# adi-gov-tw/Taiwan-Tongues-ASR-CE

Measured on AMD Instinct MI355X. Metric: audio-sec/s (RTF) whisper-large-v3 greedy, 30 s clips, batch 32; 1/2/4/8 GPU, higher is better.
Workload: dtype bf16

## Files before the change

taiwan_tongues_asr_ce_amd/csrc/common.hpp:

```cpp
#pragma once
#include <hip/hip_runtime.h>
#include <stdint.h>

typedef uint16_t bf16_t;

using f32x4 = __attribute__((ext_vector_type(4))) float;
using f32x16 = __attribute__((ext_vector_type(16))) float;
using s16x8 = __attribute__((ext_vector_type(8))) short;
using s16x4 = __attribute__((ext_vector_type(4))) short;

__device__ __forceinline__ float bf2f(bf16_t v) { return __uint_as_float(((uint32_t)v) << 16); }
__device__ __forceinline__ bf16_t f2bf(float f) { return __builtin_bit_cast(bf16_t, (__bf16)f); }
__device__ __forceinline__ uint32_t f2bf_pk(float lo, float hi) {
  typedef __bf16 bf16x2_hw __attribute__((ext_vector_type(2)));
  typedef float f32x2_hw __attribute__((ext_vector_type(2)));
  return __builtin_bit_cast(uint32_t, __builtin_convertvector((f32x2_hw){lo, hi}, bf16x2_hw));
}
struct f16_t { uint16_t bits; };
using h16x8 = __attribute__((ext_vector_type(8))) _Float16;
typedef _Float16 h16x2_hw __attribute__((ext_vector_type(2)));

template <typename T> struct N16;
template <> struct N16<bf16_t> {
  static __device__ __forceinline__ float up(uint16_t b) { return __uint_as_float(((uint32_t)b) << 16); }
// ... 198 lines not shown
                const float* filters , const float* dft_cos, const float* dft_sin ,
                const float* window , float* logmel , unsigned* clip_max ,
                hipStream_t s, const int64_t* geom_dev = nullptr);
unsigned mel_max_to_ordered(float v);
float mel_max_from_ordered(unsigned u);
template <typename T>
void launch_mel_finish(float* logmel, const unsigned* clip_max, T* mel_t , int B, int n_mels,
                       int n_frames, hipStream_t s, const int64_t* geom_dev = nullptr);
template <typename T>
void launch_mel_transpose(const float* mel, T* mel_t, int B, int n_mels, int n_frames, hipStream_t s);

template <typename T> void launch_enc_attn_simple(const T* qkv, T* out, int B, int T_, int H, hipStream_t s);
template <typename T16> void launch_enc_attn_flash_bf16(const T16* qkv, T16* out, int B, int T_, int H, hipStream_t s);
template <typename T16>
void launch_cross_attn_flash_bf16(const T16* q, const T16* K, const T16* V, T16* out, int n_clips, int n_q, int H, int Tk, hipStream_t s);

struct RuleDyn { int32_t max_prompt, max_new, sot_index; uint32_t seed; };
struct DecState {
  int32_t* cur_tok;
  int32_t* step;
  int32_t* n_sampled;
  int32_t* last_tok;
  int32_t* pen_tok;
  int32_t* last_ts;
  int32_t* done;
  int32_t* n_done;
  float* sum_logprob;
  float* no_speech;
  int32_t* out_tokens;
  const int32_t* prompt;
  const int32_t* prompt_len;
  const uint8_t* mask;
  const RuleDyn* dyn;
  const int32_t* row_cap;
};
struct RuleParams {
  int V, ldv, max_prompt, max_new;
  int eot, no_timestamps, timestamp_begin, no_speech, sot_index, timestamps, max_initial, suppress_eot;
  float temperature;
  uint32_t seed;
};
template <typename T>
void launch_cross_attn_probs(const T* q, const T* K, const T* V, T* out, int rows, int H, int Tk, const int* sel ,
                             float* probs , hipStream_t s);
void launch_token_logprob(const float* logits, int ldv, int V, const int32_t* target, float* out, int rows, hipStream_t s);
void launch_token_prob(const float* logits, int ldv, int V, int tok, float* out , int rows, hipStream_t s);
template <typename T>
void launch_embed_prefill(const int32_t* prompt, int max_prompt, int rows_per_prompt, int n_seq, int npos, const T* emb, const T* pos,
                          float* x, int d, hipStream_t s);
template <typename T>
void launch_self_attn_prefill(const T* qkv , T* kv_pool, const int32_t* page_table, int pages_per_seq,
                              int64_t pool_layer_off, int identity_pages, T* out, int n_seq, int npos, int H, hipStream_t s);
template <typename T>
void launch_self_attn_decode(const T* qkv , T* kv_pool, const int32_t* page_table, int pages_per_seq,
                             int64_t pool_layer_off, int identity_pages, int row0, const int32_t* step, T* out , int B, int H,
                             hipStream_t s, SlabIn sq = SlabIn{} ,
                             const int32_t* done = nullptr );
template <typename T>
void launch_self_attn_decode_rows(const T* qkv, T* kv_pool, const int32_t* page_table, int pages_per_seq, int64_t pool_layer_off,
                                  int identity_pages, int row0, const int32_t* row_pos, T* out, int B, int H, hipStream_t s, SlabIn sq,
                                  const int32_t* done);
template <typename T>
void launch_copy_pages(T* pool, const int32_t* pairs_dev, int n_pairs, int n_layers, int H, int64_t layer_elems, hipStream_t s);
template <typename T>
void launch_cross_attn_decode(const T* q , const T* K, const T* V , T* out, int B, int H,
                              int Tk, int kv_div, hipStream_t s,
                              float* split_ws = nullptr ,
                              SlabIn sq = SlabIn{} ,
                              int ws_rows = 0 ,
                              QProj qp = QProj{} ,
                              const int32_t* done = nullptr );
template <typename T> void launch_xkv_quant(const T* src, uint8_t* dst, float* scale, int64_t n_blocks, int rows, hipStream_t s);
template <typename T>
bool launch_cross_attn_fp8(const T* q, const uint8_t* K8, const uint8_t* V8, const float* kscale, const float* vscale, T* out, int B, int H,
                           int Tk, hipStream_t s, struct SlabIn sq, const int32_t* done = nullptr);
extern thread_local bool g_kernel_sig_on;
extern thread_local char g_kernel_sig[192];
template <typename T> inline const char* sig_type() { return sizeof(T) == 4 ? "float" : "unsigned short"; }
template <> inline const char* sig_type<struct f16_t>() { return "f16_t"; }

extern thread_local char g_launch_fault[160];
void launch_fault(const char* fmt, ...);
extern thread_local int g_skinny_x_lds;
extern thread_local int g_skinny_nt;
extern thread_local int g_xattn_variant;
extern thread_local int g_flash_qw;
extern thread_local int g_xattn_mq_slices;
extern thread_local int g_xattn_deep_items;
struct BeamRowState { const int32_t *n_sampled, *last_tok, *pen_tok, *last_ts; const uint8_t* mask; };
void launch_beam_topk(const float* logits, BeamRowState st, RuleParams rp, int R, int k, float* out_lp ,
                      int32_t* out_id , float* out_no_speech , hipStream_t s);
void launch_select(const float* logits, DecState st, RuleParams rp, int B, float* out_rows , hipStream_t s,
                   int32_t* ticket, int total_rows);
void launch_advance(int32_t* step, hipStream_t s);
void launch_select_rows(const float* logits, DecState st, RuleParams rp, int B, hipStream_t s);
void launch_admit_rows(const int32_t* tab, int n, int B, int max_prompt, DecState st, int32_t* prompt, int32_t* prompt_len, int32_t* row_cap,
                       int32_t* row_pos, hipStream_t s);
void launch_prep_weight(const void* src, int src_type , float* dst, int64_t n, int64_t conv_in, float scale,
                        hipStream_t s);
template <typename T> void launch_cast(const float* in, T* out, int64_t n, hipStream_t s);
template <typename T> void launch_uncast(const T* in, float* out, int64_t n, hipStream_t s);
```

taiwan_tongues_asr_ce_amd/csrc/engine_ctx.hpp:

```cpp
#pragma once
#include <hip/hip_runtime.h>

#include <cmath>
#include <cstdarg>
#include <cstdio>
#include <cstdlib>
#include <cstring>
#include <algorithm>
#include <atomic>
#include <map>
#include <memory>
#include <mutex>
#include <string>
#include <unordered_map>
#include <vector>

#include "../../include/ttasr.h"
#include "common.hpp"

namespace ttasr_detail {


extern thread_local std::string g_create_error;

// ... 24 lines not shown
  int device = 0;
  hipStream_t stream = nullptr;
  hipStream_t cur = nullptr;
  std::string err;
  bool lowp = false;
  bool f16 = false;
  bool finalized = false;
  bool force_basic = false;
  bool use_graph = true;
  size_t esz = 4;
  int T = 0, F = 0, d = 0, H = 0, ffn = 0, V = 0, ldv = 0, M = 0, maxB = 0, n_samples = 0;
  int pages_per_seq = 0;
  std::vector<void*> allocs;
  struct Pool { char* base = nullptr; size_t cap = 0, used = 0; } small_pool, big_pool;
  size_t arena_hint = 0;
  std::unordered_map<std::string, Slot> slots;

  void *conv1_w = nullptr, *conv2_w = nullptr, *emb = nullptr, *dpos = nullptr, *emb_sh = nullptr;
  float *conv1_b = nullptr, *conv2_b = nullptr, *epos = nullptr, *elnf_g = nullptr, *elnf_b = nullptr, *dlnf_g = nullptr,
        *dlnf_b = nullptr;
  std::vector<EncLayerW> enc;
  std::vector<DecLayerW> dec;
  float* stage_f32 = nullptr;
  float* stage_raw = nullptr;
  size_t stage_elems = 0;

  float *filters = nullptr, *dcos = nullptr, *dsin = nullptr, *window = nullptr;

  float* pcm_dev = nullptr; int64_t* nsamp_dev = nullptr; unsigned* clip_max = nullptr; int64_t* mel_geom = nullptr;
  float* mel = nullptr; void* mel_t = nullptr; void* c1 = nullptr;
  float* x = nullptr; void *h = nullptr, *qkv = nullptr, *att = nullptr, *mid = nullptr, *enc_out = nullptr;
  void* xkv = nullptr; int64_t xkv_layer_elems = 0, xkv_which_elems = 0;
  bool xkv_fp8 = false, xkv8_valid = false; uint8_t* xkv8 = nullptr; float* xkv8_scale = nullptr;
  void* pool = nullptr; int64_t pool_layer_elems = 0; int32_t* page_table = nullptr;
  float* xsplit_ws = nullptr;
  float* dx = nullptr; void *dh = nullptr, *dqkv = nullptr, *dq = nullptr, *datt = nullptr, *dmid = nullptr; float* logits = nullptr;
  float* rows_out = nullptr;
  int kv_div = 1;
  int identity_pages = 1;
  int32_t* pairs_dev = nullptr;
  float* topk_lp = nullptr; int32_t* topk_id = nullptr; int32_t* row_state = nullptr;
#ifdef TTASR_EXPERIMENTS
  int skip_mask = 0;
#else
  static constexpr int skip_mask = 0;
#endif
  float* slab = nullptr;
  int ks_want[4] = {0, 0, 0, 0};
  int gemm_force = 0;
  bool gemm_persistent = true;
  bool vocab_persistent = true;
  bool no_flash = false;
  int prefill_ns_min = 2;
  bool enc_res_epilogue = false;
  DecState st{}; int32_t* prompt_dev = nullptr; int32_t* plen_dev = nullptr; uint8_t* mask_dev = nullptr;
  ttasr_ctx* weight_owner = nullptr;
  std::atomic<int> sharers{0};
  bool destroy_pending = false;
  int32_t* row_cap_dev = nullptr;
  int flash_qw = 2;
  int xattn_mq_slices = 0;
  int xattn_deep_items = 512;
  bool ragged_exit = true;
  RuleDyn* rule_dyn_dev = nullptr; RuleDyn rule_dyn_host{};
  int32_t* pinned_i32 = nullptr;
  char* pinned_beam = nullptr; size_t pinned_beam_bytes = 0;
  float beam_prof_ms[4]{0, 0, 0, 0};
  int max_new_alloc = 0, max_prompt_alloc = 0;

  ttasr_detail::Session* sess = nullptr;
  bool session_rows = false;
  bool refill_overlap = false;
  int32_t* row_pos = nullptr;
  void* xkv_stage = nullptr;
  int32_t* admit_dev = nullptr;

  int B_mel = 0, B_enc = 0, B_dec = 0;
  std::atomic_flag busy = ATOMIC_FLAG_INIT;
  int xattn_nt = 1, xattn_pipe = 1, weights_nt = 1;
  bool dec_narrow = true;
  bool weights_packed = false;
  bool enc_ln_defer = true;
  bool dec_x_lds = true;
  bool gemm_tail = true;
  bool xkv_grouped = true;
  bool multi_step = true;
  bool no_xsplit = false;
  bool no_prefill = false;
  bool prefill_tiled = false;
  hipEvent_t ev[8]{};
  std::string bench_sig;
  float phase_ms[4]{0, 0, 0, 0};
  bool enc_timing = false;
  std::vector<hipEvent_t> enc_ev;
  std::vector<int> enc_ev_class;
  float enc_class_ms[8]{0, 0, 0, 0, 0, 0, 0, 0};

  struct GraphKey { int B; int mode; int variant; hipGraphExec_t exec; };
  std::vector<GraphKey> graphs;
  static constexpr size_t kMaxGraphs = 32;
  RuleParams rp{};
};

namespace ttasr_detail {

int fail(ttasr_ctx* c, int code, const char* fmt, ...);

#define HIPCHK(c, call)                                                                                       \
  do {                                                                                                        \
    hipError_t e_ = (call);                                                                                   \
    if (e_ != hipSuccess) return fail((c), TTASR_E_HIP, "%s failed: %s (%s:%d)", #call, hipGetErrorString(e_), \
                                      __FILE__, __LINE__);                                                    \
  } while (0)


template <class F>
inline int guarded(ttasr_ctx* c, F&& f) {
  struct Busy {
    ttasr_ctx* c; bool own;
    explicit Busy(ttasr_ctx* c_) : c(c_), own(c_ == nullptr || !c_->busy.test_and_set(std::memory_order_acquire)) {}
    ~Busy() { if (c && own) c->busy.clear(std::memory_order_release); }
  } busy(c);
  if (!busy.own) return TTASR_E_INVALID;
  if (c) { g_xattn_variant = c->xattn_nt | (c->xattn_pipe << 1); g_skinny_nt = c->weights_nt; g_skinny_narrow = c->dec_narrow ? 1 : 0; g_skinny_x_lds = c->dec_x_lds ? 1 : 0; g_xattn_deep_items = c->xattn_deep_items; g_xattn_mq_slices = c->xattn_mq_slices; g_flash_qw = c->flash_qw; }
  g_launch_fault[0] = 0;
  try {
    const int rc = f();
    if (g_launch_fault[0] && rc == TTASR_OK) return fail(c, TTASR_E_INVALID, "launcher refused: %s", g_launch_fault);
    return rc;
  } catch (const std::bad_alloc&) {
    return fail(c, TTASR_E_NOMEM, "host allocation failed");
  } catch (const std::exception& e) {
    return fail(c, TTASR_E_INVALID, "C++ exception: %s", e.what());
  } catch (...) {
    return fail(c, TTASR_E_INVALID, "unknown C++ exception");
  }
}

template <typename P>
int dalloc(ttasr_ctx* c, P** p, size_t bytes, bool zero = true) {
  if (bytes == 0) bytes = 16;
  bytes = (bytes + 255) & ~(size_t)255;
  ttasr_ctx::Pool& pool = bytes < (1u << 20) ? c->small_pool : c->big_pool;
  const size_t big_chunk = c->arena_hint >= ((size_t)1 << 30) ? (size_t)1 << 30 : (size_t)64 << 20;
  const size_t chunk = &pool == &c->small_pool ? (size_t)64 << 20 : big_chunk;
  if (bytes > chunk / 2) {
    void* q = nullptr;
    hipError_t e = hipMalloc(&q, bytes);
    if (e != hipSuccess) return fail(c, TTASR_E_NOMEM, "hipMalloc(%zu) failed: %s", bytes, hipGetErrorString(e));
    c->allocs.push_back(q);
    if (zero) HIPCHK(c, hipMemsetAsync(q, 0, bytes, c->stream));
    *p = (P*)q;
    return 0;
  }
  if (pool.used + bytes > pool.cap) {
    void* q = nullptr;
    hipError_t e = hipMalloc(&q, chunk);
    if (e != hipSuccess) return fail(c, TTASR_E_NOMEM, "hipMalloc(%zu) failed: %s", chunk, hipGetErrorString(e));
    c->allocs.push_back(q);
    pool.base = (char*)q; pool.cap = chunk; pool.used = 0;
  }
  void* q = pool.base + pool.used;
  pool.used += bytes;
  if (zero) HIPCHK(c, hipMemsetAsync(q, 0, bytes, c->stream));
  *p = (P*)q;
  return 0;
}
#define TRY(expr) do { int rc_ = (expr); if (rc_ != 0) return rc_; } while (0)
#define TT_DISPATCH(c_, CALL)                                   \
  do {                                                          \
    if (!(c_)->lowp) { using T = float; CALL; }                 \
    else if ((c_)->f16) { using T = f16_t; CALL; }              \
    else { using T = bf16_t; CALL; }                            \
  } while (0)

template <typename T>
GemmArgs lin_args(const void* A, const void* W, int M, int N, int K) {
  GemmArgs g; g.A = A; g.W = W; g.M = M; g.N = N; g.K = K; g.lda = K; g.ldw = K; g.epi.ldc = N;
  return g;
}

enum EncClass { EC_CONV = 0, EC_LN = 1, EC_QKV = 2, EC_ATTN = 3, EC_OUT = 4, EC_FC1 = 5, EC_FC2 = 6, EC_XKV = 7 };
struct AlignOut {
  int clip;
  const int* sel;
  float* probs;
};

int build_weights(ttasr_ctx* c);
int build_workspaces(ttasr_ctx* c);
int ingest_tensor(ttasr_ctx* c, const char* name, const void* src, int src_type, const int64_t* dims, int32_t ndim);

void enc_mark(ttasr_ctx* c, int cls);
void sched_encoder(ttasr_ctx* c, int B);
void sched_cross_kv(ttasr_ctx* c, int B);
void sched_prefill(ttasr_ctx* c, int n_seq, int npos, int seq_per_clip, int max_prompt, const AlignOut* al = nullptr);
int sched_prefill_no_speech(ttasr_ctx* c, int n_seq, int npos, int sot, int no_speech_tok);
void sched_gemm(ttasr_ctx* c, const GemmArgs& g);
void sched_dec_gemm(ttasr_ctx* c, const GemmArgs& g, const void* Wsh);
int prefill_positions(const ttasr_ctx* c, int min_plen, const ttasr_gen_opts* o, bool ns_from_prefill = false);
int step_graph(ttasr_ctx* c, int B, int mode, int nsteps = 1);
void drop_graphs(ttasr_ctx* c);
void drop_rule_graphs(ttasr_ctx* c);

int session_refusal(ttasr_ctx* c);
void session_free(ttasr_ctx* c);

// ... 19 lines not shown
```

taiwan_tongues_asr_ce_amd/csrc/engine_search.hip:

```cpp
#include "engine_ctx.hpp"
#include <chrono>

namespace ttasr_detail {

int check_ready(ttasr_ctx* c, int B) {
  if (!c) return TTASR_E_INVALID;
  if (!c->finalized) return fail(c, TTASR_E_INVALID, "weights not finalized (call ttasr_finalize_weights first)");
  TRY(session_refusal(c));
  if (B < 1 || B > c->maxB) return fail(c, TTASR_E_INVALID, "batch %d outside [1, max_batch=%d]", B, c->maxB);
  HIPCHK(c, hipSetDevice(c->device));
  return 0;
}

int upload_rules(ttasr_ctx* c, const ttasr_gen_opts* o, int max_prompt) {
  if (!o) return fail(c, TTASR_E_INVALID, "opts is NULL");
  if (o->max_new_tokens < 1 || o->max_new_tokens > c->max_new_alloc)
    return fail(c, TTASR_E_INVALID, "max_new_tokens %d outside [1, %d]", o->max_new_tokens, c->max_new_alloc);
  std::vector<uint8_t> mask(c->V, 0);
  for (int i = 0; i < o->n_suppress; ++i) {
    int t = o->suppress[i];
    if (t < 0 || t >= c->V) return fail(c, TTASR_E_INVALID, "suppress id %d outside vocabulary", t);
    mask[t] |= 1;
  }
  for (int i = 0; i < o->n_begin_suppress; ++i) {
    int t = o->begin_suppress[i];
    if (t < 0 || t >= c->V) return fail(c, TTASR_E_INVALID, "begin_suppress id %d outside vocabulary", t);
    mask[t] |= 2;
  }
  HIPCHK(c, hipMemcpyAsync(c->mask_dev, mask.data(), c->V, hipMemcpyHostToDevice, c->stream));
  HIPCHK(c, hipStreamSynchronize(c->stream));
  RuleParams& rp = c->rp;
  rp.V = c->V; rp.ldv = c->ldv; rp.max_prompt = max_prompt; rp.max_new = o->max_new_tokens;
  rp.eot = o->eot; rp.no_timestamps = o->no_timestamps; rp.timestamp_begin = o->timestamp_begin;
  rp.no_speech = o->no_speech; rp.sot_index = o->sot_index; rp.timestamps = o->timestamps;
  rp.max_initial = o->max_initial_timestamp_index; rp.suppress_eot = o->suppress_eot;
  rp.temperature = 0.f; rp.seed = 0;
  if (rp.eot < 0 || rp.eot >= c->V || rp.timestamp_begin < 0 || rp.timestamp_begin > c->V)
    return fail(c, TTASR_E_INVALID, "special token ids outside vocabulary");
  return 0;
}

int commit_rules(ttasr_ctx* c, const RuleParams& old) {
  c->rule_dyn_host = RuleDyn{c->rp.max_prompt, c->rp.max_new, c->rp.sot_index, c->rp.seed};
  HIPCHK(c, hipMemcpyAsync(c->rule_dyn_dev, &c->rule_dyn_host, sizeof(RuleDyn), hipMemcpyHostToDevice, c->stream));
  RuleParams a = old;
  a.max_prompt = c->rp.max_prompt; a.max_new = c->rp.max_new; a.sot_index = c->rp.sot_index; a.seed = c->rp.seed;
  if (memcmp(&a, &c->rp, sizeof a) != 0) drop_rule_graphs(c);
  return 0;
}

int set_option(ttasr_ctx* c, const std::string& key, int v) {
  const bool on = v != 0;
  if (key == "enc_kernel_timing") { c->enc_timing = on; return 0; }
  if (key == "refill_overlap") { c->refill_overlap = on; return 0; }
  if (key == "flash") c->no_flash = !on;
  else if (key == "prefill") c->no_prefill = !on;
  else if (key == "vocab_persistent") c->vocab_persistent = on;
  else if (key == "xsplit") c->no_xsplit = !on;
  else if (key == "graph") c->use_graph = on;
  else if (key == "multi_step_graph") c->multi_step = on;
  else if (key == "generic_kernels") c->force_basic = on;
  else if (key == "prefill_tiled") c->prefill_tiled = on;
  else if (key == "prefill_ns_min") { if (v < 0) return 1; c->prefill_ns_min = v; }
  else if (key == "enc_residual_epilogue") c->enc_res_epilogue = on;
  else if (key == "enc_gemm") { if (v < 0 || v > 4) return 1; c->gemm_force = v; }
  else if (key == "enc_gemm_persistent") c->gemm_persistent = on;
  else if (key == "xkv_grouped") c->xkv_grouped = on;
  else if (key == "enc_gemm_tail") c->gemm_tail = on;
  else if (key == "enc_ln_defer") c->enc_ln_defer = on;
  else if (key == "dec_narrow_blocks") { if (c->weights_packed && on != c->dec_narrow) return 1; c->dec_narrow = on; }
  else if (key == "ksplit_out") { if (v < 0 || v > 16) return 1; c->ks_want[0] = v; }
  else if (key == "ksplit_q") { if (v < 0 || v > 16) return 1; c->ks_want[1] = v; }
  else if (key == "ksplit_qkv") { if (v < 0 || v > 16) return 1; c->ks_want[2] = v; }
  else if (key == "ksplit_fc2") { if (v < 0 || v > 16) return 1; c->ks_want[3] = v; }
  else if (key == "xattn_nontemporal") c->xattn_nt = on ? 1 : 0;
  else if (key == "xattn_pipeline") c->xattn_pipe = on ? 1 : 0;
  else if (key == "xkv_fp8") {
    if (on && !c->lowp) return 1;
    if (on && (!c->xkv8 || !c->xkv8_scale)) {
      const size_t n = (size_t)c->cfg.dec_layers * c->xkv_layer_elems;
      if (!c->xkv8_scale && dalloc(c, &c->xkv8_scale, (size_t)c->cfg.dec_layers * 2 * c->maxB * c->H * sizeof(float)) != 0) return 2;
      if (!c->xkv8 && dalloc(c, &c->xkv8, n, false) != 0) return 2;
    }
    c->xkv_fp8 = on; c->xkv8_valid = false;
  }
  else if (key == "weights_nontemporal") c->weights_nt = on ? 1 : 0;
  else if (key == "dec_x_lds") c->dec_x_lds = on;
  else if (key == "ragged_exit") c->ragged_exit = on;
  else if (key == "flash_qw") { if (v < 1 || v > 2) return 1; c->flash_qw = v; }
  else if (key == "xattn_mq_slices") { if (v < 0 || v > 8) return 1; c->xattn_mq_slices = v; }
  else if (key == "xattn_deep_items") { if (v < 0 || v > 1 << 20) return 1; c->xattn_deep_items = v; }
  else return 1;
  g_xattn_variant = c->xattn_nt | (c->xattn_pipe << 1); g_skinny_nt = c->weights_nt; g_skinny_narrow = c->dec_narrow ? 1 : 0;
  g_skinny_x_lds = c->dec_x_lds ? 1 : 0;
  g_xattn_deep_items = c->xattn_deep_items; g_xattn_mq_slices = c->xattn_mq_slices; g_flash_qw = c->flash_qw;
  drop_graphs(c);
  return 0;
}

int reset_search(ttasr_ctx* c, int B) {
  hipStream_t s = c->stream;
  HIPCHK(c, hipMemsetAsync(c->st.step, 0, 16, s));
  HIPCHK(c, hipMemsetAsync(c->st.n_sampled, 0, B * 4, s));
  HIPCHK(c, hipMemsetAsync(c->st.last_tok, 0xff, B * 4, s));
  HIPCHK(c, hipMemsetAsync(c->st.pen_tok, 0xff, B * 4, s));
  HIPCHK(c, hipMemsetAsync(c->st.last_ts, 0xff, B * 4, s));
  HIPCHK(c, hipMemsetAsync(c->st.done, 0, B * 4, s));
  HIPCHK(c, hipMemsetAsync(c->st.n_done, 0, 16, s));
  HIPCHK(c, hipMemsetAsync(c->st.sum_logprob, 0, B * 4, s));
  HIPCHK(c, hipMemsetAsync(c->st.no_speech, 0, B * 4, s));
  HIPCHK(c, hipMemsetAsync(c->row_cap_dev, 0x7f, B * 4, s));
  return 0;
}

int generate_rows(ttasr_ctx* c, int R, int rows_per_clip, const int32_t* prompt, const int32_t* prompt_len, int max_prompt,
                  const ttasr_gen_opts* o, float temperature, uint32_t seed, int32_t* out_tokens, int32_t* out_len, float* out_lp,
                  float* out_ns, const int32_t* row_cap) {
  int min_plen = 1 << 30, max_plen = 0;
  const int A = R / rows_per_clip;
  for (int a = 0; a < A; ++a) {
    if (prompt_len[a] < 1 || prompt_len[a] > max_prompt) return fail(c, TTASR_E_INVALID, "prompt_len[%d]=%d", a, prompt_len[a]);
    if (prompt_len[a] >= c->cfg.n_text_ctx)
      return fail(c, TTASR_E_INVALID, "prompt_len[%d]=%d leaves no room in the %d-token context", a, prompt_len[a], c->cfg.n_text_ctx);
    min_plen = std::min(min_plen, prompt_len[a]); max_plen = std::max(max_plen, prompt_len[a]);
    for (int j = 0; j < prompt_len[a]; ++j)
      if (prompt[a * max_prompt + j] < 0 || prompt[a * max_prompt + j] >= c->V)
        return fail(c, TTASR_E_INVALID, "prompt token outside vocabulary");
  }
  RuleParams old = c->rp;
  TRY(upload_rules(c, o, max_prompt));
  c->rp.temperature = temperature; c->rp.seed = seed;
  TRY(commit_rules(c, old));
  TRY(reset_search(c, R));
  hipStream_t s = c->stream;
  std::vector<int32_t> pr((size_t)R * max_prompt, 0), pl(R);
  for (int r = 0; r < R; ++r) {
    const int a = r / rows_per_clip;
    pl[r] = prompt_len[a];
    memcpy(&pr[(size_t)r * max_prompt], &prompt[(size_t)a * max_prompt], (size_t)max_prompt * 4);
  }
  HIPCHK(c, hipMemcpyAsync(c->prompt_dev, pr.data(), pr.size() * 4, hipMemcpyHostToDevice, s));
  HIPCHK(c, hipMemcpyAsync(c->plen_dev, pl.data(), R * 4, hipMemcpyHostToDevice, s));
  HIPCHK(c, hipMemcpy2DAsync(c->st.cur_tok, 4, c->prompt_dev, (size_t)max_prompt * 4, 4, R, hipMemcpyDeviceToDevice, s));
  int max_cap = o->max_new_tokens;
  if (row_cap) {
    max_cap = 1;
    for (int r = 0; r < R; ++r) {
      if (row_cap[r] < 1 || row_cap[r] > o->max_new_tokens)
        return fail(c, TTASR_E_INVALID, "row_max_new[%d]=%d outside [1, max_new_tokens=%d]", r, row_cap[r], o->max_new_tokens);
      max_cap = std::max(max_cap, (int)row_cap[r]);
    }
    HIPCHK(c, hipMemcpyAsync(c->row_cap_dev, row_cap, (size_t)R * 4, hipMemcpyHostToDevice, s));
  }
  HIPCHK(c, hipStreamSynchronize(s));
  c->st.prompt = c->prompt_dev; c->st.prompt_len = c->plen_dev;
  c->B_dec = R;
  c->kv_div = rows_per_clip;
  struct Restore { ttasr_ctx* c; ~Restore() { c->kv_div = 1; } } restore{c};
  const int interval = std::max(1, o->check_interval);
  const int last_step = std::min(c->cfg.n_text_ctx - 1, max_plen - 1 + max_cap);
  hipEventRecord(c->ev[5], s);
  const int pre = prefill_positions(c, min_plen, o, min_plen - 1 >= c->prefill_ns_min);
  if (pre > 0) {
    sched_prefill(c, R, pre, rows_per_clip, max_prompt);
    if (o->no_speech >= 0 && o->sot_index < pre) {
      TRY(sched_prefill_no_speech(c, R, pre, o->sot_index, o->no_speech));
    }
    c->pinned_i32[1] = pre;
    HIPCHK(c, hipMemcpyAsync(c->st.step, &c->pinned_i32[1], 4, hipMemcpyHostToDevice, s));
    HIPCHK(c, hipMemcpy2DAsync(c->st.cur_tok, 4, c->prompt_dev + pre, (size_t)max_prompt * 4, 4, R, hipMemcpyDeviceToDevice, s));
  }
  for (int step = pre; step < last_step; ++step) {
    const bool all_forced = step + 1 < min_plen;
    const bool need_logits = !all_forced || (o->no_speech >= 0 && step == o->sot_index);
    int run = 1;
    if (c->multi_step && need_logits && step + 1 >= min_plen) {
      int until_poll = last_step - step;
// ... 279 lines not shown
```

taiwan_tongues_asr_ce_amd/csrc/kernels_skinny.hip:

```cpp
#include "common.hpp"
#include <mutex>
#include <cstdlib>
using u32x4 = __attribute__((ext_vector_type(4))) unsigned;

thread_local int g_skinny_narrow = 1;
int skinny_rows_per_block(int N, int K) {
  (void)K;
  if (!g_skinny_narrow) return 32;
  return (N % 20 == 0 && (N / 20) % 256 == 0) ? 20 : 32;
}

template <typename T16>
__global__ void shuffle_cast_kernel(const float* __restrict__ src, bf16_t* __restrict__ dst, int rows, int K, int row_offset, int rpb) {
  const int ks_per = K / 16, per = 2 * rpb;
  const int n_blocks = (rows + rpb - 1) / rpb;
  const int64_t n_chunks = (int64_t)n_blocks * ks_per * per;
  for (int64_t c = (int64_t)blockIdx.x * blockDim.x + threadIdx.x; c < n_chunks; c += (int64_t)gridDim.x * blockDim.x) {
    const int within = (int)(c % per);
    const int64_t blk = c / per;
    const int ks = (int)(blk % ks_per), nb = (int)(blk / ks_per);
    const int half = within / rpb, lr = within - half * rpb;
    const int r = nb * rpb + lr;
    if (r >= rows) continue;
    const float* s = src + (int64_t)r * K + ks * 16 + 8 * half;
// ... 143 lines not shown
  } else {
    prefetch_epilogue();
    for (int i0 = 0; i0 < steps; i0 += U) {
      u32x4 w[U], xv[RB][U];
#pragma unroll
      for (int u = 0; u < U; ++u) {
        const int i = min(i0 + u, steps - 1);
        if constexpr (NT) w[u] = __builtin_nontemporal_load(wp + (int64_t)i * wstep); else w[u] = wp[(int64_t)i * wstep];
      }
#pragma unroll
      for (int g = 0; g < RB; ++g)
#pragma unroll
        for (int u = 0; u < U; ++u) xv[g][u] = *(const u32x4*)(xp[g] + min(i0 + u, steps - 1) * 16);
#pragma unroll
      for (int u = 0; u < U; ++u)
        if (i0 + u < steps) {
#pragma unroll
          for (int g = 0; g < RB; ++g)
            acc[g] = N16<T16>::mfma32(*(s16x8*)&w[u], *(s16x8*)&xv[g][u], acc[g]);
        }
    }
  }
#pragma unroll
  for (int g = 0; g < RB; ++g)
#pragma unroll
    for (int q = 0; q < 4; ++q)
      *(float4*)&red[wave][g][(lane & 31) * 32 + 8 * q + 4 * (lane >> 5)] =
          make_float4(acc[g][4 * q], acc[g][4 * q + 1], acc[g][4 * q + 2], acc[g][4 * q + 3]);
  __syncthreads();
  if (!ecell) return;
#pragma unroll
  for (int g = 0; g < RB; ++g) {
    float4 v = *(const float4*)&red[0][g][(tid >> 3) * 32 + 4 * (tid & 7)];
#pragma unroll
    for (int w = 1; w < NW; ++w) {
      const float4 t = *(const float4*)&red[w][g][(tid >> 3) * 32 + 4 * (tid & 7)];
      v.x += t.x; v.y += t.y; v.z += t.z; v.w += t.w;
    }
    v.x += ebias.x; v.y += ebias.y; v.z += ebias.z; v.w += ebias.w;
    const int b = g * 32 + (tid >> 3);
    if (b >= B) continue;
    float vv[4] = {v.x, v.y, v.z, v.w};
    const float rr[4] = {eres[g].x, eres[g].y, eres[g].z, eres[g].w};
    const int64_t idx0 = (int64_t)b * e.ldc + en;
    if (en + 3 < N && ksplit > 1) {
      *(float4*)(slab + (int64_t)ks * slab_stride + idx0) = v;
      continue;
    }
    if (en + 3 < N && ksplit == 1) {
#pragma unroll
      for (int j = 0; j < 4; ++j) {
        if (e.act == 1) vv[j] = gelu_erf(vv[j]);
        if (e.residual) vv[j] += rr[j];
      }
      if (e.out_f32) *(float4*)(e.out_f32 + idx0) = make_float4(vv[0], vv[1], vv[2], vv[3]);
      if (e.out_t) {
        uint2 pk;
        pk.x = N16<T16>::pk(vv[0], vv[1]);
        pk.y = N16<T16>::pk(vv[2], vv[3]);
        *(uint2*)((bf16_t*)e.out_t + idx0) = pk;
      }
      continue;
    }
#pragma unroll
    for (int j = 0; j < 4; ++j) {
      const int n = en + j;
      if (n < N) {
        const int64_t idx = idx0 + j;
        if (ksplit > 1) {
          slab[(int64_t)ks * slab_stride + idx] = vv[j];
        } else {
          float o = vv[j];
          if (e.bias) o += e.bias[n];
          if (e.act == 1) o = gelu_erf(o);
          if (e.residual) o += e.residual[idx];
          if (e.out_f32) e.out_f32[idx] = o;
          if (e.out_t) ((bf16_t*)e.out_t)[idx] = N16<T16>::down(o);
        }
      }
    }
  }
}

template <typename T16, int RB, bool NT>
__global__ __launch_bounds__(512) void gemm_vocab_kernel(const bf16_t* __restrict__ Wsh_, const bf16_t* __restrict__ x_, int B_, int N_,
                                                         int K_, int steps_, float* __restrict__ out_, int64_t ldc_) {
  constexpr int NW = 8, U = 10;
  extern __shared__ __attribute__((aligned(16))) float vred[];
  const bf16_t* Wsh = sgpr_pin_ptr(Wsh_);
  const bf16_t* x = sgpr_pin_ptr(x_);
  const int B = sgpr_pin(B_), N = sgpr_pin(N_), K = sgpr_pin(K_), steps = sgpr_pin(steps_);
  float* out = sgpr_pin_ptr(out_);
  const int64_t ldc = sgpr_pin(ldc_);
  const int tid = threadIdx.x, lane = tid & 63, wave = tid >> 6;
  const int ks_per = K / 16, n_blocks = (N + 31) / 32;
  const int k0 = wave * steps;
  const u32x4* wbase = (const u32x4*)Wsh + (int64_t)k0 * 64 + lane;
  auto load_w = [&](int nb, u32x4 (&w)[U]) {
    const u32x4* wp = wbase + (int64_t)min(nb, n_blocks - 1) * ks_per * 64;
#pragma unroll
    for (int u = 0; u < U; ++u) {
      const int i = min(u, steps - 1);
      if constexpr (NT) w[u] = __builtin_nontemporal_load(wp + (int64_t)i * 64); else w[u] = wp[(int64_t)i * 64];
    }
  };
  int nb = blockIdx.x;
  u32x4 wa[U], wb[U];
  load_w(nb, wa);
  u32x4 xv[RB][U];
#pragma unroll
  for (int g = 0; g < RB; ++g) {
    const bf16_t* xp = x + (int64_t)min(g * 32 + (lane & 31), B - 1) * K + k0 * 16 + 8 * (lane >> 5);
#pragma unroll
    for (int u = 0; u < U; ++u) xv[g][u] = *(const u32x4*)(xp + min(u, steps - 1) * 16);
  }
  int par = 0;
  auto block = [&](int nb_cur, u32x4 (&wc)[U], u32x4 (&wn)[U]) {
    load_w(nb_cur + gridDim.x, wn);
    f32x16 acc[RB];
#pragma unroll
    for (int g = 0; g < RB; ++g)
#pragma unroll
      for (int j = 0; j < 16; ++j) acc[g][j] = 0.f;
#pragma unroll
    for (int u = 0; u < U; ++u)
      if (u < steps) {
#pragma unroll
        for (int g = 0; g < RB; ++g) acc[g] = N16<T16>::mfma32(*(s16x8*)&wc[u], *(s16x8*)&xv[g][u], acc[g]);
      }
    float* red = vred + (size_t)par * NW * RB * 1024;
#pragma unroll
    for (int g = 0; g < RB; ++g)
#pragma unroll
      for (int q = 0; q < 4; ++q)
        *(float4*)&red[(wave * RB + g) * 1024 + (lane & 31) * 32 + 8 * q + 4 * (lane >> 5)] =
            make_float4(acc[g][4 * q], acc[g][4 * q + 1], acc[g][4 * q + 2], acc[g][4 * q + 3]);
    __syncthreads();
    if (tid < 256) {
      const int en = nb_cur * 32 + 4 * (tid & 7);
#pragma unroll
      for (int g = 0; g < RB; ++g) {
        float4 v = *(const float4*)&red[(0 * RB + g) * 1024 + (tid >> 3) * 32 + 4 * (tid & 7)];
#pragma unroll
        for (int w = 1; w < NW; ++w) {
          const float4 t = *(const float4*)&red[(w * RB + g) * 1024 + (tid >> 3) * 32 + 4 * (tid & 7)];
          v.x += t.x; v.y += t.y; v.z += t.z; v.w += t.w;
        }
        const int b = g * 32 + (tid >> 3);
        if (b < B) {
          float* o = out + (int64_t)b * ldc + en;
          if (en + 3 < N) *(float4*)o = v;
          else { const float vv[4] = {v.x, v.y, v.z, v.w};
#pragma unroll
            for (int j = 0; j < 4; ++j) if (en + j < N) o[j] = vv[j]; }
        }
      }
    }
    par ^= 1;
  };
  while (nb < n_blocks) {
    block(nb, wa, wb);
    nb += gridDim.x;
    if (nb >= n_blocks) break;
    block(nb, wb, wa);
    nb += gridDim.x;
  }
}

static int g_vocab_cus[64] = {0};
static std::once_flag g_vocab_once[64];
static void vocab_init_once(int device);
void gemm_vocab_init(int device) { std::call_once(g_vocab_once[device & 63], vocab_init_once, device); }
static void vocab_init_once(int device) {
  hipDeviceProp_t p;
  g_vocab_cus[device & 63] = hipGetDeviceProperties(&p, device) == hipSuccess ? p.multiProcessorCount : 256;
#define TTASR_VOCAB_ATTR(T_, RB_)                                                                                                          \
  hipFuncSetAttribute((const void*)gemm_vocab_kernel<T_, RB_, true>, hipFuncAttributeMaxDynamicSharedMemorySize, 2 * 8 * RB_ * 4096);     \
  hipFuncSetAttribute((const void*)gemm_vocab_kernel<T_, RB_, false>, hipFuncAttributeMaxDynamicSharedMemorySize, 2 * 8 * RB_ * 4096)
  TTASR_VOCAB_ATTR(bf16_t, 1); TTASR_VOCAB_ATTR(bf16_t, 2); TTASR_VOCAB_ATTR(f16_t, 1); TTASR_VOCAB_ATTR(f16_t, 2);
#undef TTASR_VOCAB_ATTR
}

template <typename T16>
bool launch_gemm_vocab(const T16* Wsh, const T16* x, int B, int N, int K, float* out, int64_t ldc, hipStream_t s, int device) {
  const int n_cu = g_vocab_cus[device & 63];
  if (n_cu <= 0 || B < 1 || B > 64 || K % 128 != 0 || K / 128 > 10 || N < 8192 || ldc % 4 != 0) return false;
  if (skinny_rows_per_block(N, K) != 32) return false;
  const int rb = (B + 31) / 32, steps = K / 128, n_blocks = (N + 31) / 32;
  const int grid = n_blocks < n_cu ? n_blocks : n_cu;
  const size_t lds = (size_t)2 * 8 * rb * 1024 * sizeof(float);
#define TTASR_VOCAB(RB_)                                                                                                           \
  do {                                                                                                                             \
    if (g_skinny_nt) hipLaunchKernelGGL((gemm_vocab_kernel<T16, RB_, true>), dim3(grid), dim3(512), lds, s, (const bf16_t*)Wsh, (const bf16_t*)x, B, N, K, steps, out, ldc); \
    else hipLaunchKernelGGL((gemm_vocab_kernel<T16, RB_, false>), dim3(grid), dim3(512), lds, s, (const bf16_t*)Wsh, (const bf16_t*)x, B, N, K, steps, out, ldc); \
  } while (0)
  if (rb == 1) TTASR_VOCAB(1); else TTASR_VOCAB(2);
#undef TTASR_VOCAB
  return true;
}
template bool launch_gemm_vocab<bf16_t>(const bf16_t*, const bf16_t*, int, int, int, float*, int64_t, hipStream_t, int);
template bool launch_gemm_vocab<f16_t>(const f16_t*, const f16_t*, int, int, int, float*, int64_t, hipStream_t, int);

int gemm_skinny_ksplit(int B, int N, int K, int want) {
  if (B < 1 || B > 128 || K % 64 != 0) return 1;
  const int rpb = skinny_rows_per_block(N, K);
  const int rb = (B + 31) / 32, n_blocks = (N + rpb - 1) / rpb, ks_per = K / 16;
  const int per4 = ks_per / 4;
  if (ks_per % 4 != 0) return 1;
  int best = 1;
  if (want > 0) {
    for (int s = 1; s <= want && s <= 16; ++s) if (per4 % s == 0) best = s;
    return best;
  }
  const int u_max = rb == 1 ? 10 : (rb == 2 ? 8 : 5);
  for (int s = 1; s <= 16; ++s) {
    if (per4 % s != 0) continue;
    best = s;
    const int steps = per4 / s;
    if (steps <= u_max && ((steps <= 10 && n_blocks * s >= 256) || (steps <= 5 && n_blocks * s >= 160))) break;
  }
  return best;
}

template <typename T16>
bool launch_gemm_skinny(const T16* Wsh_, const T16* x_, int B, int N, int K, const GemmEpi& e, hipStream_t s, int ksplit,
                        float* slab, int64_t slab_stride) {
  const bf16_t* Wsh = (const bf16_t*)Wsh_;
  const bf16_t* x = (const bf16_t*)x_;
  if (B < 1 || B > 128 || K % 64 != 0 || e.rowtab || e.headsplit) return false;
  const int rb = (B + 31) / 32;
  const int rpb = skinny_rows_per_block(N, K);
  const int n_blocks = (N + rpb - 1) / rpb;
  const int ks_per = K / 16;
  const int u_max = rb == 1 ? 10 : (rb == 2 ? 8 : 5);
  int nw = 4;
  if (ksplit > 1) {
    if (!slab || e.act != 0) return false;
  } else {
    ksplit = 1;
    const int nw_max = rb == 1 ? 16 : 8;
    while (nw < nw_max && ks_per % (nw * 2) == 0 && ks_per / nw > u_max) nw *= 2;
    if (nw < 8 && ks_per % 8 == 0 && ks_per / 8 >= 5 && n_blocks < 256) nw = 8;
  }
  if (ks_per % (nw * ksplit) != 0) return false;
  const int steps = ks_per / (nw * ksplit);
  dim3 grid(n_blocks, ksplit);
#define TTASR_SKINNY(NW_, RB_, U_, ONE_)                                                                                              \
  do {                                                                                                                                \
    const bool xl_ = g_skinny_x_lds && ONE_ && (NW_ == 4 || (NW_ == 8 && RB_ == 1));                                                  \
    const size_t lds_ = skinny_lds_bytes(NW_, RB_, steps, xl_);                                                                       \
    const int rpbx_ = rpb | (xl_ ? 256 : 0);                                                                                          \
    if (g_skinny_nt) {                                                                                                                \
      if (lds_ > 65536) skinny_allow_big_lds<gemm_skinny_kernel<T16, NW_, RB_, U_, true, ONE_>>();                                     \
      hipLaunchKernelGGL((gemm_skinny_kernel<T16, NW_, RB_, U_, true, ONE_>), grid, dim3(NW_ * 64), lds_, s, Wsh, x, B, N, K, ksplit, steps, e, slab, slab_stride, rpbx_); \
    } else {                                                                                                                          \
      if (lds_ > 65536) skinny_allow_big_lds<gemm_skinny_kernel<T16, NW_, RB_, U_, false, ONE_>>();                                    \
      hipLaunchKernelGGL((gemm_skinny_kernel<T16, NW_, RB_, U_, false, ONE_>), grid, dim3(NW_ * 64), lds_, s, Wsh, x, B, N, K, ksplit, steps, e, slab, slab_stride, rpbx_); \
    }                                                                                                                                 \
  } while (0)
#define TTASR_SKINNY_U(NW_, RB_, UMAX_)                                            \
  do {                                                                             \
    if (steps <= 2 && UMAX_ >= 2) TTASR_SKINNY(NW_, RB_, 2, true);                 \
    else if (steps <= 4 && UMAX_ >= 4) TTASR_SKINNY(NW_, RB_, 4, true);            \
    else if (steps <= 5) TTASR_SKINNY(NW_, RB_, 5, true);                          \
    else if (steps <= 8 && UMAX_ >= 8) TTASR_SKINNY(NW_, RB_, 8, true);            \
    else if (steps <= UMAX_) TTASR_SKINNY(NW_, RB_, UMAX_, true);                  \
    else TTASR_SKINNY(NW_, RB_, UMAX_, false);                                     \
  } while (0)
  if (rb == 1) {
    if (nw == 16) TTASR_SKINNY_U(16, 1, 10); else if (nw == 8) TTASR_SKINNY_U(8, 1, 10); else TTASR_SKINNY_U(4, 1, 10);
  } else if (rb == 2) {
    if (nw == 8) TTASR_SKINNY_U(8, 2, 10); else TTASR_SKINNY_U(4, 2, 8);
  } else if (rb == 3) {
    if (nw == 8) TTASR_SKINNY_U(8, 3, 10); else TTASR_SKINNY_U(4, 3, 5);
  } else {
    if (nw == 8) TTASR_SKINNY_U(8, 4, 5); else TTASR_SKINNY_U(4, 4, 5);
  }
#undef TTASR_SKINNY_U
#undef TTASR_SKINNY
  return true;
}
template bool launch_gemm_skinny<bf16_t>(const bf16_t*, const bf16_t*, int, int, int, const GemmEpi&, hipStream_t, int, float*, int64_t);
template bool launch_gemm_skinny<f16_t>(const f16_t*, const f16_t*, int, int, int, const GemmEpi&, hipStream_t, int, float*, int64_t);
```

Before: 2159.

## Add wide skinny GEMM kernel packing several column blocks per workgroup

Adds a decoder skinny GEMM variant that processes G (2 or 4) weight column blocks per workgroup, sharing a single LDS-staged copy of the activation rows across the groups. The default selects it automatically when the batch spans at least two 32-row blocks and the grid would otherwise exceed 256 blocks. The aim is to reuse activations across column blocks and cut redundant x loads and the block count. In exchange it needs more LDS and larger workgroups, which may lower occupancy.

Result: no change. 2161, median of 3 (+0.1%).

```diff
diff --git a/taiwan_tongues_asr_ce_amd/csrc/common.hpp b/taiwan_tongues_asr_ce_amd/csrc/common.hpp
--- a/taiwan_tongues_asr_ce_amd/csrc/common.hpp
+++ b/taiwan_tongues_asr_ce_amd/csrc/common.hpp
@@ -304,6 +304,7 @@
 extern thread_local char g_launch_fault[160];
 void launch_fault(const char* fmt, ...);
 extern thread_local int g_skinny_x_lds;
+extern thread_local int g_skinny_wide;
 extern thread_local int g_skinny_nt;
 extern thread_local int g_xattn_variant;
 extern thread_local int g_flash_qw;
diff --git a/taiwan_tongues_asr_ce_amd/csrc/engine_ctx.hpp b/taiwan_tongues_asr_ce_amd/csrc/engine_ctx.hpp
--- a/taiwan_tongues_asr_ce_amd/csrc/engine_ctx.hpp
+++ b/taiwan_tongues_asr_ce_amd/csrc/engine_ctx.hpp
@@ -130,6 +130,7 @@
   bool weights_packed = false;
   bool enc_ln_defer = true;
   bool dec_x_lds = true;
+  int dec_wide = 1;
   bool gemm_tail = true;
   bool xkv_grouped = true;
   bool multi_step = true;
@@ -170,7 +171,7 @@
     ~Busy() { if (c && own) c->busy.clear(std::memory_order_release); }
   } busy(c);
   if (!busy.own) return TTASR_E_INVALID;
-  if (c) { g_xattn_variant = c->xattn_nt | (c->xattn_pipe << 1); g_skinny_nt = c->weights_nt; g_skinny_narrow = c->dec_narrow ? 1 : 0; g_skinny_x_lds = c->dec_x_lds ? 1 : 0; g_xattn_deep_items = c->xattn_deep_items; g_xattn_mq_slices = c->xattn_mq_slices; g_flash_qw = c->flash_qw; }
+  if (c) { g_xattn_variant = c->xattn_nt | (c->xattn_pipe << 1); g_skinny_nt = c->weights_nt; g_skinny_narrow = c->dec_narrow ? 1 : 0; g_skinny_x_lds = c->dec_x_lds ? 1 : 0; g_skinny_wide = c->dec_wide; g_xattn_deep_items = c->xattn_deep_items; g_xattn_mq_slices = c->xattn_mq_slices; g_flash_qw = c->flash_qw; }
   g_launch_fault[0] = 0;
   try {
     const int rc = f();
diff --git a/taiwan_tongues_asr_ce_amd/csrc/engine_search.hip b/taiwan_tongues_asr_ce_amd/csrc/engine_search.hip
--- a/taiwan_tongues_asr_ce_amd/csrc/engine_search.hip
+++ b/taiwan_tongues_asr_ce_amd/csrc/engine_search.hip
@@ -86,13 +86,14 @@
   }
   else if (key == "weights_nontemporal") c->weights_nt = on ? 1 : 0;
   else if (key == "dec_x_lds") c->dec_x_lds = on;
+  else if (key == "dec_wide_gemm") { if (v < 0 || v > 4 || v == 3) return 1; c->dec_wide = v; }
   else if (key == "ragged_exit") c->ragged_exit = on;
   else if (key == "flash_qw") { if (v < 1 || v > 2) return 1; c->flash_qw = v; }
   else if (key == "xattn_mq_slices") { if (v < 0 || v > 8) return 1; c->xattn_mq_slices = v; }
   else if (key == "xattn_deep_items") { if (v < 0 || v > 1 << 20) return 1; c->xattn_deep_items = v; }
   else return 1;
   g_xattn_variant = c->xattn_nt | (c->xattn_pipe << 1); g_skinny_nt = c->weights_nt; g_skinny_narrow = c->dec_narrow ? 1 : 0;
-  g_skinny_x_lds = c->dec_x_lds ? 1 : 0;
+  g_skinny_x_lds = c->dec_x_lds ? 1 : 0; g_skinny_wide = c->dec_wide;
   g_xattn_deep_items = c->xattn_deep_items; g_xattn_mq_slices = c->xattn_mq_slices; g_flash_qw = c->flash_qw;
   drop_graphs(c);
   return 0;
diff --git a/taiwan_tongues_asr_ce_amd/csrc/kernels_skinny.hip b/taiwan_tongues_asr_ce_amd/csrc/kernels_skinny.hip
--- a/taiwan_tongues_asr_ce_amd/csrc/kernels_skinny.hip
+++ b/taiwan_tongues_asr_ce_amd/csrc/kernels_skinny.hip
@@ -249,6 +249,202 @@
   }
 }
 
+thread_local int g_skinny_wide = 1;
+template <int G, int RB>
+struct SkinnyWidePlan {
+  static constexpr int RP = G * 4 * RB * 4096 <= 128 * 1024 ? RB : 2;
+  static size_t lds_bytes(int steps) {
+    const size_t tile = (size_t)RB * 32 * ((size_t)4 * steps * 32 + 16);
+    return std::max(tile, (size_t)G * 4 * RP * 4096);
+  }
+};
+
+template <typename T16, int RB, int U, bool NT, int G>
+__global__ __launch_bounds__(G * 256) void gemm_skinny_wide_kernel(const bf16_t* __restrict__ Wsh_, const bf16_t* __restrict__ x_,
+                                                                   int B_, int N_, int K_, int ksplit_, int steps_, GemmEpi e,
+                                                                   float* __restrict__ slab_, int64_t slab_stride_, int rpb_) {
+  constexpr int NW = 4;
+  constexpr int RP = SkinnyWidePlan<G, RB>::RP;
+  extern __shared__ __attribute__((aligned(16))) char smem[];
+  float (*red)[NW][RP][32 * 32] = (float (*)[NW][RP][32 * 32])smem;
+  const bf16_t* Wsh = sgpr_pin_ptr(Wsh_);
+  const bf16_t* x = sgpr_pin_ptr(x_);
+  const int B = sgpr_pin(B_), N = sgpr_pin(N_), K = sgpr_pin(K_), ksplit = sgpr_pin(ksplit_);
+  const int rpb = sgpr_pin(rpb_);
+  const int steps = sgpr_pin(steps_);
+  float* slab = sgpr_pin_ptr(slab_);
+  const int64_t slab_stride = sgpr_pin(slab_stride_);
+  e.bias = sgpr_pin_ptr(e.bias); e.residual = sgpr_pin_ptr(e.residual); e.out_f32 = sgpr_pin_ptr(e.out_f32);
+  e.out_t = sgpr_pin_ptr(e.out_t); e.ldc = sgpr_pin(e.ldc); e.act = sgpr_pin(e.act);
+  const int tid = threadIdx.x, lane = tid & 63, wave = (tid >> 6) & (NW - 1), gi = tid >> 8, ltid = tid & 255;
+  const int nb = blockIdx.x * G + gi, ks = blockIdx.y;
+  const bool live = nb * rpb < N;
+  const int nbw = live ? nb : blockIdx.x * G;
+  const int ks_per = K / 16;
+  const int k0 = (ks * NW + wave) * steps;
+  const int wstep = 2 * rpb;
+  const u32x4* wp = (const u32x4*)Wsh + ((int64_t)nbw * ks_per + k0) * wstep + (lane >> 5) * rpb + min(lane & 31, rpb - 1);
+  const int en = nb * rpb + 4 * (ltid & 7);
+  const bool ecell = live && 4 * (ltid & 7) < rpb;
+  float4 ebias = make_float4(0.f, 0.f, 0.f, 0.f), eres[RB];
+#pragma unroll
+  for (int g = 0; g < RB; ++g) eres[g] = ebias;
+  f32x16 acc[RB];
+#pragma unroll
+  for (int g = 0; g < RB; ++g)
+#pragma unroll
+    for (int j = 0; j < 16; ++j) acc[g][j] = 0.f;
+  constexpr int TPR = 2 * NW;
+  constexpr int RPP = G * 32;
+  constexpr int NP = (RB * 32 + RPP - 1) / RPP;
+  const int xrow = tid / TPR, xcq = tid % TPR;
+  const int stride = NW * steps * 32 + 16;
+  u32x4 w[U], xr[NP][U];
+#pragma unroll
+  for (int p = 0; p < NP; ++p) {
+    const bf16_t* xg = x + (int64_t)min(p * RPP + xrow, B - 1) * K + (int64_t)(ks * NW * steps) * 16 + xcq * 8;
+#pragma unroll
+    for (int u = 0; u < U; ++u) xr[p][u] = *(const u32x4*)(xg + min(u, steps - 1) * TPR * 8);
+  }
+  if (ecell && en + 3 < N) {
+    if (e.bias && ksplit == 1) ebias = *(const float4*)(e.bias + en);
+    if (e.residual && ksplit == 1) {
+#pragma unroll
+      for (int g = 0; g < RB; ++g) eres[g] = *(const float4*)(e.residual + (int64_t)min(g * 32 + (ltid >> 3), B - 1) * e.ldc + en);
+    }
+  }
+  __builtin_amdgcn_sched_barrier(0);
+#pragma unroll
+  for (int u = 0; u < U; ++u) {
+    const int i = min(u, steps - 1);
+    if constexpr (NT) w[u] = __builtin_nontemporal_load(wp + (int64_t)i * wstep); else w[u] = wp[(int64_t)i * wstep];
+  }
+  __builtin_amdgcn_sched_barrier(0);
+  asm volatile("s_waitcnt vmcnt(%0)" :: "n"(U) : "memory");
+#pragma unroll
+  for (int p = 0; p < NP; ++p)
+#pragma unroll
+    for (int u = 0; u < U; ++u)
+      if (p * RPP + xrow < RB * 32 && u < steps) *(u32x4*)(smem + (p * RPP + xrow) * stride + (u * TPR + xcq) * 16) = xr[p][u];
+  asm volatile("s_waitcnt lgkmcnt(0)" ::: "memory");
+  __builtin_amdgcn_s_barrier();
+  __builtin_amdgcn_sched_barrier(0);
+#pragma unroll
+  for (int u = 0; u < U; ++u)
+    if (u < steps) {
+#pragma unroll
+      for (int g = 0; g < RB; ++g) {
+        const u32x4 xv = *(const u32x4*)(smem + (g * 32 + (lane & 31)) * stride + ((wave * steps + u) * 2 + (lane >> 5)) * 16);
+        acc[g] = N16<T16>::mfma32(*(s16x8*)&w[u], *(const s16x8*)&xv, acc[g]);
+      }
+    }
+  __syncthreads();
+  auto store_cell = [&](int g, float4 v) {
+    v.x += ebias.x; v.y += ebias.y; v.z += ebias.z; v.w += ebias.w;
+    const int b = g * 32 + (ltid >> 3);
+    if (b >= B) return;
+    float vv[4] = {v.x, v.y, v.z, v.w};
+    const float rr[4] = {eres[g].x, eres[g].y, eres[g].z, eres[g].w};
+    const int64_t idx0 = (int64_t)b * e.ldc + en;
+    if (en + 3 < N && ksplit > 1) {
+      *(float4*)(slab + (int64_t)ks * slab_stride + idx0) = v;
+      return;
+    }
+    if (en + 3 < N && ksplit == 1) {
+#pragma unroll
+      for (int j = 0; j < 4; ++j) {
+        if (e.act == 1) vv[j] = gelu_erf(vv[j]);
+        if (e.residual) vv[j] += rr[j];
+      }
+      if (e.out_f32) *(float4*)(e.out_f32 + idx0) = make_float4(vv[0], vv[1], vv[2], vv[3]);
+      if (e.out_t) {
+        uint2 pk;
+        pk.x = N16<T16>::pk(vv[0], vv[1]);
+        pk.y = N16<T16>::pk(vv[2], vv[3]);
+        *(uint2*)((bf16_t*)e.out_t + idx0) = pk;
+      }
+      return;
+    }
+#pragma unroll
+    for (int j = 0; j < 4; ++j) {
+      const int n = en + j;
+      if (n < N) {
+        const int64_t idx = idx0 + j;
+        if (ksplit > 1) {
+          slab[(int64_t)ks * slab_stride + idx] = vv[j];
+        } else {
+          float o = vv[j];
+          if (e.bias) o += e.bias[n];
+          if (e.act == 1) o = gelu_erf(o);
+          if (e.residual) o += e.residual[idx];
+          if (e.out_f32) e.out_f32[idx] = o;
+          if (e.out_t) ((bf16_t*)e.out_t)[idx] = N16<T16>::down(o);
+        }
+      }
+    }
+  };
+#pragma unroll
+  for (int g0 = 0; g0 < RB; g0 += RP) {
+    if (g0 > 0) __syncthreads();
+#pragma unroll
+    for (int j = 0; j < RP; ++j)
+      if (g0 + j < RB)
+#pragma unroll
+        for (int q = 0; q < 4; ++q)
+          *(float4*)&red[gi][wave][j][(lane & 31) * 32 + 8 * q + 4 * (lane >> 5)] =
+              make_float4(acc[g0 + j][4 * q], acc[g0 + j][4 * q + 1], acc[g0 + j][4 * q + 2], acc[g0 + j][4 * q + 3]);
+    __syncthreads();
+    if (ecell) {
+#pragma unroll
+      for (int j = 0; j < RP; ++j)
+        if (g0 + j < RB) {
+          float4 v = *(const float4*)&red[gi][0][j][(ltid >> 3) * 32 + 4 * (ltid & 7)];
+#pragma unroll
+          for (int w2 = 1; w2 < NW; ++w2) {
+            const float4 t = *(const float4*)&red[gi][w2][j][(ltid >> 3) * 32 + 4 * (ltid & 7)];
+            v.x += t.x; v.y += t.y; v.z += t.z; v.w += t.w;
+          }
+          store_cell(g0 + j, v);
+        }
+    }
+  }
+}
+
+static int skinny_wide_groups(int rb, int n_blocks, int ksplit) {
+  if (rb < 2 || !g_skinny_wide || !g_skinny_x_lds) return 0;
+  if (g_skinny_wide == 2 || g_skinny_wide == 4) return g_skinny_wide;
+  if (rb == 3 || n_blocks * ksplit <= 256) return 0;
+  for (int g = 2; g <= 4; g *= 2)
+    if ((n_blocks + g - 1) / g * ksplit <= 256) return g;
+  return 0;
+}
+
+template <typename T16, int RB, int U, bool NT, int G>
+static void launch_skinny_wide_g(const bf16_t* Wsh, const bf16_t* x, int B, int N, int K, const GemmEpi& e, hipStream_t s, int ksplit,
+                                 int steps, float* slab, int64_t slab_stride, int rpb, int n_blocks) {
+  const size_t lds = SkinnyWidePlan<G, RB>::lds_bytes(steps);
+  if (lds > 65536) skinny_allow_big_lds<gemm_skinny_wide_kernel<T16, RB, U, NT, G>>();
+  hipLaunchKernelGGL((gemm_skinny_wide_kernel<T16, RB, U, NT, G>), dim3((n_blocks + G - 1) / G, ksplit), dim3(G * 256), lds, s, Wsh, x,
+                     B, N, K, ksplit, steps, e, slab, slab_stride, rpb);
+}
+template <typename T16, int NW, int RB, int U, bool ONE>
+static bool launch_skinny_wide(int G, const bf16_t* Wsh, const bf16_t* x, int B, int N, int K, const GemmEpi& e, hipStream_t s,
+                               int ksplit, int steps, float* slab, int64_t slab_stride, int rpb, int n_blocks) {
+  if constexpr (NW == 4 && RB >= 2 && ONE) {
+#define TTASR_WIDE(G_)                                                                                                               \
+  do {                                                                                                                               \
+    if (g_skinny_nt) launch_skinny_wide_g<T16, RB, U, true, G_>(Wsh, x, B, N, K, e, s, ksplit, steps, slab, slab_stride, rpb, n_blocks);   \
+    else launch_skinny_wide_g<T16, RB, U, false, G_>(Wsh, x, B, N, K, e, s, ksplit, steps, slab, slab_stride, rpb, n_blocks);              \
+  } while (0)
+    if (G == 2) { TTASR_WIDE(2); return true; }
+    if (G == 4) { TTASR_WIDE(4); return true; }
+#undef TTASR_WIDE
+  }
+  (void)G; (void)Wsh; (void)x; (void)B; (void)N; (void)K; (void)e; (void)s; (void)ksplit; (void)steps; (void)slab; (void)slab_stride;
+  (void)rpb; (void)n_blocks;
+  return false;
+}
+
 template <typename T16, int RB, bool NT>
 __global__ __launch_bounds__(512) void gemm_vocab_kernel(const bf16_t* __restrict__ Wsh_, const bf16_t* __restrict__ x_, int B_, int N_,
                                                          int K_, int steps_, float* __restrict__ out_, int64_t ldc_) {
@@ -412,8 +608,11 @@
   if (ks_per % (nw * ksplit) != 0) return false;
   const int steps = ks_per / (nw * ksplit);
   dim3 grid(n_blocks, ksplit);
+  const int wide_g = skinny_wide_groups(rb, n_blocks, ksplit);
 #define TTASR_SKINNY(NW_, RB_, U_, ONE_)                                                                                              \
   do {                                                                                                                                \
+    if (wide_g && launch_skinny_wide<T16, NW_, RB_, U_, ONE_>(wide_g, Wsh, x, B, N, K, e, s, ksplit, steps, slab, slab_stride, rpb,   \
+                                                              n_blocks)) break;                                                       \
     const bool xl_ = g_skinny_x_lds && ONE_ && (NW_ == 4 || (NW_ == 8 && RB_ == 1));                                                  \
     const size_t lds_ = skinny_lds_bytes(NW_, RB_, steps, xl_);                                                                       \
     const int rpbx_ = rpb | (xl_ ? 256 : 0);                                                                                          \
```
